# UZ-SLAMLab/DefSLAM

Measured on AMD Instinct MI355X. Metric: SfT GN iters/sec (500-node mesh, 1k matches), higher is better.
Workload: dtype f64

## Files before the change

### defslam_amd/csrc/sft_batch.h

```cpp
#pragma once

#define SFTB_NW 8
#ifndef SFTB_LIN_NW
#define SFTB_LIN_NW 8
#endif
#ifndef SFTB_LIN_WAVES
#define SFTB_LIN_WAVES 2
#endif
#ifndef SFTB_TRIAL_WAVES
#define SFTB_TRIAL_WAVES 2
#endif

__device__ __forceinline__ void sftb_ctl_lds(char* smem, Ctl*& ctl, double*& red, double*& out, double*& panel) {
  ctl = reinterpret_cast<Ctl*>(smem);
  red = reinterpret_cast<double*>(smem + 512);
  out = red + 16 * 27 + 5;
  panel = out + 32;
}

__global__ __launch_bounds__(64 * SFTB_NW, 2) void sftb_init_kernel(const SftDev* __restrict__ probs, SftRun* __restrict__ runs, int* __restrict__ counters, int* __restrict__ lin_list, int tail_below) {
  const SftDev& P = probs[blockIdx.x];
  if (blockIdx.x == 0 && threadIdx.x == 0 && (int)gridDim.x <= tail_below) counters[6] = 1;
  init_state<64 * SFTB_NW>(P);
  if (threadIdx.x == 0) {
    SftRun& R = runs[blockIdx.x];
    R.lambda = -1.0; R.ni = 2.0; R.chi_cur = 0.0; R.chi_ini = 0.0; R.rho = 0.0; R.lambda_start = 0.0;
    R.it = 0; R.qmax = 0; R.nbad = 0; R.accepted = 0; R.all_ok = 1; R.iters = 0; R.trials = 0; R.fact_ok = 1;
    R.state = P.max_iters > 0 ? SFTB_LIN : SFTB_FINISH;
    if (P.max_iters > 0) lin_list[atomicAdd(&counters[2], 1)] = blockIdx.x;
  }
}

template <int NW>
__device__ __forceinline__ void sftb_lin_problem(const SftDev& P, SftRun& R, Ctl* ctl, double* red, double* out, double* panel) {
  constexpr int NT = 64 * NW;
  const int tid = threadIdx.x;
  auto nothing = [] {};
  const double chi0 = linearise<NW, decltype(nothing), true>(P, ctl, red, out, panel, nothing);
  double lambda = R.lambda;
  if (R.it == 0) {
    double mx = 0.0;
    for (int r = tid; r < P.Dn; r += NT) mx = fmax(mx, fabs(h_diag(P, r)));
    if (tid < 6) mx = fmax(mx, fabs(P.Hcorner[tid * 8]));
    mx = block_max(mx, red);
    lambda = 1e-5 * mx;
  }
  if (tid == 0) {
    if (R.it == 0) { R.lambda = lambda; R.ni = 2.0; R.nbad = 0; }
    R.chi_cur = chi0; R.chi_ini = chi0; R.qmax = 0; R.rho = 0.0; R.accepted = 0; R.all_ok = 1; R.lambda_start = lambda;
    R.state = SFTB_TRIAL;
  }
}

__global__ __launch_bounds__(64 * SFTB_LIN_NW, SFTB_LIN_WAVES) void sftb_lin_kernel(const SftDev* __restrict__ probs, SftRun* __restrict__ runs, int* __restrict__ counters,
                                                                                  const int* __restrict__ lin_list, int B, int tail_below) {
  constexpr int NW = SFTB_LIN_NW, NT = 64 * NW;
  extern __shared__ __attribute__((aligned(16))) char smem[];
  __shared__ int next_b;
  Ctl* ctl; double *red, *out, *panel;
  sftb_ctl_lds(smem, ctl, red, out, panel);
  const int tid = threadIdx.x;
  if (counters[6] || B - counters[0] <= tail_below) {
    if (blockIdx.x == 0 && tid == 0) counters[6] = 1;
    return;
  }
  if (blockIdx.x == 0 && tid == 0) counters[7]++;
  auto fetch = [&]() { const int i = atomicAdd(&counters[3], 1); return i < counters[2] ? lin_list[i] : -1; };
  int nxt = -1;
  if (tid == 0) nxt = fetch();
  while (true) {
    if (tid == 0) next_b = nxt;
    __syncthreads();
    const int b = __builtin_amdgcn_readfirstlane(next_b);
    if (b < 0) break;
    if (tid == 0) { nxt = fetch(); atomicAdd(&counters[9], 1); }
    sftb_lin_problem<NW>(probs[b], runs[b], ctl, red, out, panel);
  }
}

__global__ __launch_bounds__(64, 1) void sftb_factor_kernel(const SftDev* __restrict__ probs, SftRun* __restrict__ runs, int* __restrict__ counters, int B) {
  extern __shared__ __attribute__((aligned(16))) char smem[];
  lds_double* lds = to_lds(reinterpret_cast<double*>(smem));
  const int lane = threadIdx.x;
  if (counters[6]) return;
  for (int i = lane; i < WV_LDS_DOUBLES; i += 64) lds[i] = 0.0;
  if (blockIdx.x == 0 && lane == 0) { counters[2] = 0; counters[3] = 0; }
  WvPrev Q;
  Q.Lg = nullptr; Q.Linv = nullptr; Q.x = nullptr; Q.nT = 0; Q.active = 0; Q.xb = 0.0;
  int n_done = 0;
  while (true) {
    int b = 0;
    if (lane == 0) b = atomicAdd(&counters[1], 1);
    b = __builtin_amdgcn_readfirstlane(b);
    if (b >= B) break;
    if (runs[b].state != SFTB_TRIAL) continue;
    const SftDev& P = probs[b];
    const double lambda = runs[b].lambda;
    double xcam;
    const int ok = wv_factor(P, lambda, lambda, lds, Q, xcam);
    if (lane == 0) runs[b].fact_ok = ok;
    Q = wv_prev_of(P, ok, xcam, lane);
    n_done++;
  }
  int lane_now;
  asm volatile("v_mbcnt_lo_u32_b32 %0, -1, 0\n\tv_mbcnt_hi_u32_b32 %0, -1, %0" : "=v"(lane_now));
  if (Q.active) wv_backsub_now(Q, lane_now);
  if (lane_now == 0 && n_done) atomicAdd(&counters[8], n_done);
}

template <int NW>
__device__ __forceinline__ int sftb_trial_problem(const SftDev& P, SftRun& R, Ctl* ctl, double* red, double* out, double* panel, int* counters, int* lin_list, int b) {
  constexpr int NT = 64 * NW;
  const int tid = threadIdx.x;
  const int Dn = P.Dn;
  const int Dnp = ((Dn + NB - 1) / NB) * NB;
  const int ok = R.fact_ok;
  const double lam = R.lambda;
  const bool in_lds = P.lds_class >= 1;
  if (!in_lds)
    for (int i = tid; i < 3 * P.n; i += NT) {
      const double v = P.xyz[i];
      P.xyz_bak[i] = v;
      const int a = P.act[i / 3];
      if (a >= 0) P.xyz[i] = v + P.x[3 * a + (i % 3)];
    }
  if (tid < 7) R.pose_bak[tid] = P.pose[tid];
  __syncthreads();
  if (tid == 0) pose_oplus(P.pose, P.x + Dnp);
  double sc = 0.0;
  for (int r = tid; r < Dn; r += NT) { const double xv = P.x[r]; sc += xv * (lam * xv + P.Hbord[(size_t)6 * Dnp + r]); }
  if (tid < 6) { const double xv = P.x[Dnp + tid]; sc += xv * (lam * xv + P.Hcorner[42 + tid]); }
  __syncthreads();
  block_sum<1>(&sc, red, out);
  const double scale = out[0];
  __syncthreads();
  const auto staged = asm_records<NW, 1>(P, panel);
  const double chi_new = in_lds ? eval_edges<false, 1>(P, ctl, red, out, staged, P.x)
                                : eval_edges<false, 0>(P, ctl, red, out, asm_records<NW, 0>(P, panel));
  if (tid == 0) {
    const double tempChi = ok ? chi_new : DBL_MAX;
    double rho = (R.chi_cur - tempChi);
    rho /= (scale + 1e-3);
    R.rho = rho;
    if (rho > 0 && isfinite(tempChi)) {
      double alpha = 1. - pow((2 * rho - 1), 3);
      alpha = fmin(alpha, 2. / 3.);
      const double sf = fmax(1. / 3., alpha);
      R.lambda = lam * sf; R.ni = 2.0; R.chi_cur = tempChi; R.accepted = 1;
      ctl->stop = 0;
    } else {
      R.lambda = lam * R.ni; R.ni *= 2.0;
      ctl->stop = 1;
    }
    R.qmax++;
    R.all_ok &= ok;
    ctl->qmax = R.qmax;
    ctl->rho = rho;
  }
  __syncthreads();
  if (ctl->stop) {
    if (!in_lds)
      for (int i = tid; i < 3 * P.n; i += NT) P.xyz[i] = P.xyz_bak[i];
    if (tid < 7) P.pose[tid] = R.pose_bak[tid];
  } else if (in_lds) {
    for (int i = tid; i < 3 * P.n; i += NT) P.xyz[i] = staged.xyz_l[i];
  }
  const bool again = (ctl->rho < 0) && (ctl->qmax < 10);
  if (again) return 0;
  __syncthreads();
  if (tid == 0) {
    const int qmax = R.qmax;
// ... 101 lines not shown
```

### defslam_amd/csrc/sft_wave.h

```cpp
#pragma once

#if defined(WV_STEP_TRACE) && defined(DSH_LAB)
#define WV_T_DECL long long wv_tr[9] = {0, 0, 0, 0, 0, 0, 0, 0, 0}, wv_tl = clock64()
#define WV_T(e) do { const long long t__ = clock64(); wv_tr[e] += t__ - wv_tl; wv_tl = t__; } while (0)
#define WV_T_ARG , long long (&wv_tr)[9], long long& wv_tl
#define WV_T_PASS , wv_tr, wv_tl
#define WV_T_DUMP(P) do { if ((threadIdx.x & 63) == 0) for (int e__ = 0; e__ < 9; e__++) (P).dbg[40 + e__] = (double)wv_tr[e__]; } while (0)
#else
#define WV_T_DECL do {} while (0)
#define WV_T(e) do {} while (0)
#define WV_T_ARG
#define WV_T_PASS
#define WV_T_DUMP(P) do {} while (0)
#endif

__host__ __device__ constexpr int wv_phys(int r, int d) {
  return d == 0 ? r : (d <= 3 ? 8 * d + r : (d == 4 ? 32 + (r & 3) : 8 * (8 - d) + ((r + 8 - d) & 7)));
}
constexpr int WV_AGPR_TILES = 32;
constexpr int WV_L_WIN = 0;
constexpr int WV_L_BORD = 1024;
constexpr int WV_L_WSCR = 2048;
constexpr int WV_L_CN = 2336;
constexpr int WV_L_XRING = 2400;
// ... 145 lines not shown
struct WvB2 { double n0, n1; };
struct WvBO { double v[4][2]; };
__device__ __forceinline__ WvB2 wv_bq_load(const lds_double* tile, int lane) {
  const v2d_w a = reinterpret_cast<const lds_v2d*>(tile)[lane];
  return WvB2{a.x, a.y};
}
__device__ __forceinline__ void wv_bq_store(lds_double* tile, int lane, const WvB2& v) {
  reinterpret_cast<lds_v2d*>(tile)[lane] = (v2d_w){v.n0, v.n1};
}
__device__ __forceinline__ int wv_bo_lane(int lane) { return (lane & 0x30) | (lane & 3); }
__device__ __forceinline__ void wv_bo_load(const lds_double* tile, int lane, WvBO& o) {
  const lds_v2d* p = reinterpret_cast<const lds_v2d*>(tile) + wv_bo_lane(lane);
#pragma unroll
  for (int q = 0; q < 4; q++) { const v2d_w a = p[4 * q]; o.v[q][0] = a.x; o.v[q][1] = a.y; }
}
__device__ __forceinline__ void wv_upd_b4(WvB2& C, const v4d& A, const WvBO& B, int q0 = 0) {
#define WV_MF(q) asm volatile("v_mfma_f64_4x4x4_4b_f64 %0, %2, %3, %0 neg:[1,0,0]\n\tv_mfma_f64_4x4x4_4b_f64 %1, %2, %4, %1 neg:[1,0,0]" \
                              : "+v"(C.n0), "+v"(C.n1) : "v"(A[q]), "v"(B.v[q][0]), "v"(B.v[q][1]) : "memory")
  asm volatile("s_nop 1" : "+v"(C.n0), "+v"(C.n1));
  if (q0 <= 0) WV_MF(0);
  if (q0 <= 1) WV_MF(1);
  if (q0 <= 2) WV_MF(2);
  WV_MF(3);
#undef WV_MF
}
__device__ __forceinline__ void wv_trsm_b4(WvB2& Y, const v4d& Wt, const WvBO& B) {
  asm volatile("s_nop 1\n\t"
               "v_mfma_f64_4x4x4_4b_f64 %0, %2, %6, 0\n\t"
               "v_mfma_f64_4x4x4_4b_f64 %1, %2, %7, 0\n\t"
               "v_mfma_f64_4x4x4_4b_f64 %0, %3, %8, %0\n\t"
               "v_mfma_f64_4x4x4_4b_f64 %1, %3, %9, %1\n\t"
               "v_mfma_f64_4x4x4_4b_f64 %0, %4, %10, %0\n\t"
               "v_mfma_f64_4x4x4_4b_f64 %1, %4, %11, %1\n\t"
               "v_mfma_f64_4x4x4_4b_f64 %0, %5, %12, %0\n\t"
               "v_mfma_f64_4x4x4_4b_f64 %1, %5, %13, %1"
               : "=&v"(Y.n0), "=&v"(Y.n1)
               : "v"(Wt[0]), "v"(Wt[1]), "v"(Wt[2]), "v"(Wt[3]), "v"(B.v[0][0]), "v"(B.v[0][1]), "v"(B.v[1][0]), "v"(B.v[1][1]), "v"(B.v[2][0]), "v"(B.v[2][1]),
                 "v"(B.v[3][0]), "v"(B.v[3][1])
               : "memory");
}
__device__ __forceinline__ int wv_bstd_index(int lane) { return 2 * wv_bo_lane(lane) + ((lane >> 2) & 1); }

template <int CTRL>
__device__ __forceinline__ double wv_dpp_mov(double v) {
  const int lo = __builtin_amdgcn_mov_dpp(__double2loint(v), CTRL, 0xF, 0xF, false);
  const int hi = __builtin_amdgcn_mov_dpp(__double2hiint(v), CTRL, 0xF, 0xF, false);
  return __hiloint2double(hi, lo);
}

__device__ __forceinline__ bool wv_chol_inv(v4d& a, v4d& w) {
  const int lane = threadIdx.x & 63;
  const int g = lane >> 4, c = lane & 15;
  w = (v4d){(g == c) ? 1.0 : 0.0, (g + 4 == c) ? 1.0 : 0.0, (g + 8 == c) ? 1.0 : 0.0, (g + 12 == c) ? 1.0 : 0.0};
  double plast = 1.0;
#pragma unroll
  for (int J = 0; J < 4; J++) {
    const double aJ = a[J];
    const double sel = chol4_inverse_operand(aJ, J, g, c & 3, plast);
    const double wJ = w[J];
    double zw, lp;
    if (J < 3) {
      asm volatile("s_nop 1\n\t"
                   "v_mfma_f64_4x4x4_4b_f64 %0, %2, %3, 0\n\t"
                   "v_mfma_f64_4x4x4_4b_f64 %1, %2, %4, 0\n\t"
                   "s_nop 7"
                   : "=&v"(zw), "=&v"(lp)
                   : "v"(sel), "v"(wJ), "v"(aJ));
      const double nlp = -lp;
      const double below = (c >= 4 * J + 4) ? nlp : 0.0;
      asm volatile("s_nop 1\n\t"
                   "v_mfma_f64_16x16x4_f64 %0, %2, %3, %0\n\t"
                   "v_mfma_f64_16x16x4_f64 %1, %4, %5, %1\n\t" WV_NOP_MFMA_RESULT
                   : "+v"(a), "+v"(w)
                   : "v"(nlp), "v"(lp), "v"(below), "v"(zw));
      w[J] = zw;
    } else {
      asm volatile("s_nop 1\n\tv_mfma_f64_4x4x4_4b_f64 %0, %1, %2, 0\n\ts_nop 7" : "=&v"(zw) : "v"(sel), "v"(wJ));
      w[J] = zw;
    }
  }
  return plast > 0.0;
}

struct WvProb {
  int Dn, Dnp, nT, q8;
  double lambda, lam_corner;
  unsigned bofs;
  const SFT_G double* Hc;
  const SFT_G uint32_t* hgl;
  const SFT_G double* Hbord;
  SFT_G double *Lg, *Linv;
};

typedef unsigned v4u_w __attribute__((ext_vector_type(4)));
__device__ __forceinline__ void wv_list(const WvProb& W, int I, int d, int lane, unsigned (&o)[4]) {
  const SFT_G v4u_w* row = reinterpret_cast<const SFT_G v4u_w*>(W.hgl + ((size_t)(I < W.nT ? I : W.nT) * (BT + 1) + d) * 256);
  const v4u_w v = row[lane];
  o[0] = v.x; o[1] = v.y; o[2] = v.z; o[3] = v.w;
}
__device__ __forceinline__ v4d wv_gather_vgpr(const WvProb& W, const unsigned (&o)[4]) {
  const auto b8 = reinterpret_cast<const SFT_G char*>(W.Hc);
  v4d v;
#pragma unroll
  for (int q = 0; q < 4; q++) v[q] = *reinterpret_cast<const SFT_G double*>(b8 + o[q]);
  return v;
}
__device__ __forceinline__ WvB2 wv_border_fresh(const WvProb& W, int J, int lane) {
  const SFT_G double* p = W.Hbord + TS * (J < W.nT ? J : W.nT);
  (void)lane;
  return WvB2{p[W.bofs], p[W.bofs + 4 * (unsigned)W.Dnp]};
}

struct WvRowList { unsigned o[8][4]; };
__device__ __forceinline__ void wv_row_list(const WvProb& W, int I, int lane, WvRowList& L) {
#pragma unroll
  for (int d = 0; d < 8; d++) wv_list(W, I, d, lane, L.o[d]);
}
template <int PH, int D>
__device__ __forceinline__ void wv_row_fetch_d(const WvProb& W, const WvRowList& L, int dmax, v4d& fresh4) {
  if constexpr (D < 8) {
    if (D <= dmax) {
      if constexpr (D == 4) fresh4 = wv_gather_vgpr(W, L.o[D]);
      else wv_gather_agpr<wv_phys(PH, D)>(W.Hc, L.o[D][0], L.o[D][1], L.o[D][2], L.o[D][3]);
    }
    wv_row_fetch_d<PH, D + 1>(W, L, dmax, fresh4);
  }
}

struct WvPrev {
  const SFT_G double* Lg;
  const SFT_G double* Linv;
  SFT_G double* x;
  int nT, active;
  double xb;
};
__device__ __forceinline__ void wv_bs_request(const WvPrev& Q, int J, lds_double* land, int lane) {
  const unsigned voff = 16u * (unsigned)lane;
  const SFT_G char* col = reinterpret_cast<const SFT_G char*>(Q.Lg + ((size_t)J * (BT + 1)) * 256);
  const SFT_G char* w = reinterpret_cast<const SFT_G char*>(Q.Linv + (size_t)J * 256);
  const unsigned l0 = (unsigned)__builtin_amdgcn_readfirstlane((int)(size_t)land);
  asm volatile("s_mov_b32 m0, %2\n\ts_nop 0\n\t"
               "global_load_lds_dwordx4 %0, %1\n\t"
               "global_load_lds_dwordx4 %0, %1 offset:2048\n\t"
               "global_load_lds_dwordx4 %0, %1 offset:3072"
               :: "v"(voff), "s"(col), "s"(l0) : "memory", "m0");
#pragma unroll
  for (int grp = 1; grp < 5; grp++) {
    const SFT_G char* cg = col + 4096 * grp;
    const unsigned lg = l0 + 4096u * grp;
    if (grp < 4)
      asm volatile("s_mov_b32 m0, %2\n\ts_nop 0\n\t"
                   "global_load_lds_dwordx4 %0, %1\n\t"
                   "global_load_lds_dwordx4 %0, %1 offset:1024\n\t"
                   "global_load_lds_dwordx4 %0, %1 offset:2048\n\t"
                   "global_load_lds_dwordx4 %0, %1 offset:3072"
                   :: "v"(voff), "s"(cg), "s"(lg) : "memory", "m0");
    else
      asm volatile("s_mov_b32 m0, %2\n\ts_nop 0\n\t"
                   "global_load_lds_dwordx4 %0, %1\n\t"
                   "global_load_lds_dwordx4 %0, %1 offset:1024"
                   :: "v"(voff), "s"(cg), "s"(lg) : "memory", "m0");
  }
  asm volatile("s_mov_b32 m0, %2\n\ts_nop 0\n\t"
               "global_load_lds_dwordx4 %0, %1\n\t"
               "global_load_lds_dwordx4 %0, %1 offset:1024"
               :: "v"(voff), "s"(w), "s"(l0 + 18u * 1024u) : "memory", "m0");
}
__device__ __forceinline__ void wv_bs_column(const WvPrev& Q, int J, const lds_double* land, lds_double* xring, int lane) {
  const int c = lane & 15;
  const lds_v2d* t2 = reinterpret_cast<const lds_v2d*>(land) + 2 * lane;
  double s[4];
  {
    const lds_double* tb = land + wv_bstd_index(lane);
    s[0] = tb[0] * Q.xb; s[1] = tb[8] * Q.xb; s[2] = tb[16] * Q.xb; s[3] = tb[24] * Q.xb;
  }
#pragma unroll
  for (int d = 1; d <= 8; d++) {
    const double xr = xring[((J + d) & 7) * 16 + c];
    const v2d_w a = t2[128 * d], b = t2[128 * d + 1];
    s[0] = fma(a.x, xr, s[0]); s[1] = fma(a.y, xr, s[1]); s[2] = fma(b.x, xr, s[2]); s[3] = fma(b.y, xr, s[3]);
  }
#pragma unroll
  for (int q = 0; q < 4; q++) {
    s[q] += wv_dpp_mov<0x128>(s[q]);
    s[q] += wv_dpp_mov<0x124>(s[q]);
    s[q] += wv_dpp_mov<0x122>(s[q]);
    s[q] += wv_dpp_mov<0x121>(s[q]);
  }
  const v2d_w wa = t2[128 * 9], wb = t2[128 * 9 + 1];
  double p = wa.x * -s[0];
  p = fma(wa.y, -s[1], p); p = fma(wb.x, -s[2], p); p = fma(wb.y, -s[3], p);
  p = sum_rows(p);
  if (lane < TS) { xring[(J & 7) * 16 + lane] = p; Q.x[TS * J + lane] = p; }
}
__device__ __forceinline__ void wv_bs_step(const WvPrev& Q, int J, lds_double* lds, int lane) {
  wv_bs_column(Q, J, lds + WV_L_LAND, lds + WV_L_XRING, lane);
  asm volatile("s_waitcnt lgkmcnt(0)" ::: "memory");
  if (J >= 1) wv_bs_request(Q, J - 1, lds + WV_L_LAND, lane);
}
__device__ __forceinline__ void wv_bs_begin(const WvPrev& Q, lds_double* lds, int lane) {
  lds_double* xring = lds + WV_L_XRING;
  xring[lane] = 0.0; xring[64 + lane] = 0.0;
  wv_bs_request(Q, Q.nT - 1, lds + WV_L_LAND, lane);
}
__device__ __forceinline__ void wv_backsub_now(const WvPrev& Q, int lane) {
  const int c = lane & 15;
  (void)c;
  double xr[8];
#pragma unroll
  for (int s = 0; s < 8; s++) xr[s] = 0.0;
  struct Col { v4d t[10]; };
  auto fetch = [&](int J) -> Col {
    Col C;
    if (J >= 0) {
      const SFT_G double* col = Q.Lg + ((size_t)J * (BT + 1)) * 256 + 4 * lane;
#pragma unroll
      for (int i = 1; i <= 8; i++) C.t[i] = (J + i < Q.nT) ? *reinterpret_cast<const SFT_G v4d*>(col + 256 * i) : (v4d){0.0, 0.0, 0.0, 0.0};
      {
        const SFT_G double* tb = col - 4 * lane + wv_bstd_index(lane);
        C.t[0] = (v4d){tb[0], tb[8], tb[16], tb[24]};
      }
      C.t[9] = *reinterpret_cast<const SFT_G v4d*>(Q.Linv + (size_t)J * 256 + 4 * lane);
    } else {
#pragma unroll
      for (int i = 0; i < 10; i++) C.t[i] = (v4d){0.0, 0.0, 0.0, 0.0};
    }
    return C;
  };
  auto solve_col = [&](const Col& C, int J, auto phc) {
    constexpr int ph = decltype(phc)::value;
    double s[4];
#pragma unroll
    for (int q = 0; q < 4; q++) s[q] = C.t[0][q] * Q.xb;
#pragma unroll
    for (int dd = 1; dd <= 8; dd++)
#pragma unroll
      for (int q = 0; q < 4; q++) s[q] = fma(C.t[dd][q], xr[(ph + dd) & 7], s[q]);
#pragma unroll
    for (int q = 0; q < 4; q++) {
      s[q] += wv_dpp_mov<0x128>(s[q]);
      s[q] += wv_dpp_mov<0x124>(s[q]);
      s[q] += wv_dpp_mov<0x122>(s[q]);
      s[q] += wv_dpp_mov<0x121>(s[q]);
    }
    double p = C.t[9][0] * -s[0];
#pragma unroll
    for (int q = 1; q < 4; q++) p = fma(C.t[9][q], -s[q], p);
    p = sum_rows(p);
    xr[ph] = p;
    if (lane < TS) Q.x[TS * J + lane] = p;
  };
  int J = Q.nT - 1;
  Col c0 = fetch(J), c1 = fetch(J - 1);
#pragma unroll 1
  for (; J >= 0; J -= 2) {
    const Col n0 = fetch(J - 2), n1 = fetch(J - 3);
    switch (J & 7) {
      case 7: solve_col(c0, J, std::integral_constant<int, 7>{}); solve_col(c1, J - 1, std::integral_constant<int, 6>{}); break;
      case 5: solve_col(c0, J, std::integral_constant<int, 5>{}); solve_col(c1, J - 1, std::integral_constant<int, 4>{}); break;
      case 3: solve_col(c0, J, std::integral_constant<int, 3>{}); solve_col(c1, J - 1, std::integral_constant<int, 2>{}); break;
      default: solve_col(c0, J, std::integral_constant<int, 1>{}); solve_col(c1, J - 1, std::integral_constant<int, 0>{}); break;
    }
    c0 = n0; c1 = n1;
  }
}

struct WvState {
  v4d Y[9];
  WvB2 Yq;
  WvBO Yo;
  double corner;
  v4d araw;
  WvB2 bnext;
  WvRowList rl;
  unsigned al[4];
  unsigned off_lane, off_bord;
  int ok;
};

template <int PH, int I, int IEND>
__device__ __forceinline__ void wv_trsm_cols(WvState& S, const WvTri& Wt, int k, int nT, const v4d& D4, int lane) {
  if constexpr (I <= IEND) {
    (void)k; (void)nT;
    if constexpr (I == 4) {
      wv_trsm4_vgpr(S.Y[4], Wt, D4);
    } else {
      wv_trsm4_agpr<wv_phys((PH + I) & 7, I)>(S.Y[I], Wt);
    }
    wv_trsm_cols<PH, I + 1, IEND>(S, Wt, k, nT, D4, lane);
  }
}

__host__ __device__ constexpr int wv_tile_index(int I, int J) {
  int n = 0;
  for (int i = 1; i <= 7; i++)
    for (int j = 1; j <= i; j++) {
      if (i == I && j == J) return n;
      if (i - j != 4) n++;
    }
  return n;
}
template <int PH, int SLOT>
__device__ __forceinline__ void wv_fetch_slot(const WvProb& W, const WvRowList& L) {
  if constexpr (SLOT < 28) {
    constexpr int t = SLOT / 4, q = SLOT % 4, d = t < 4 ? t : t + 1;
    wv_gather1_agpr<wv_phys(PH, d), q>(W.Hc, L.o[d][q]);
  }
}
template <int PH, bool TAIL, int I, int J>
__device__ __forceinline__ void wv_update_tiles(const WvProb& W, WvState& S, int k, int nT, int q8, SFT_G double* col) {
  if constexpr (I <= 8) {
    constexpr int d = I - J, r = (PH + I) & 7;
    if constexpr (d != 4) {
      if (!TAIL || k + I < nT) wv_upd_agpr<wv_phys(r, d)>(S.Y[J], S.Y[I], (I == 8) ? q8 : 0);
      if constexpr (I <= 7) {
        constexpr int n = wv_tile_index(I, J);
        if constexpr (n < 18) {
          const SFT_G double* slot = col + 256 * (n >> 1);
          if constexpr (n == 0) {
            const v2d_w yb = (v2d_w){S.Yq.n0, S.Yq.n1};
            asm volatile("global_store_dwordx4 %0, %1, %2" :: "v"(S.off_bord), "v"(yb), "s"(slot) : "memory");
          } else if constexpr (n >= 2) {
            const v4d& y = S.Y[n >> 1];
            const v2d_w half = (v2d_w){y[2 * (n & 1)], y[2 * (n & 1) + 1]};
            asm volatile("global_store_dwordx4 %0, %1, %2 offset:%c3" :: "v"(S.off_lane), "v"(half), "s"(slot), "n"(16 * (n & 1)) : "memory");
          }
        }
        wv_fetch_slot<PH, 2 * n>(W, S.rl);
        wv_fetch_slot<PH, 2 * n + 1>(W, S.rl);
      }
    }
    if constexpr (J < I) wv_update_tiles<PH, TAIL, I, J + 1>(W, S, k, nT, q8, col);
  }
}
template <int PH, bool TAIL, int I0, int I1>
__device__ __forceinline__ void wv_update_rows(const WvProb& W, WvState& S, int k, int nT, int q8, SFT_G double* col) {
  if constexpr (I0 <= I1) {
    wv_update_tiles<PH, TAIL, I0, 1>(W, S, k, nT, q8, col);
    wv_update_rows<PH, TAIL, I0 + 1, I1>(W, S, k, nT, q8, col);
  }
}
template <int PH, int T>
__device__ __forceinline__ lds_double* wv_task_tile(lds_double* lds) {
  if constexpr (T < 7) return lds + WV_L_BORD + 128 * ((PH + T + 1) & 7);
  else if constexpr (T < 10) return lds + WV_L_WIN + 256 * (wv_phys((PH + T - 2) & 7, 4) - WV_AGPR_TILES);
  else if constexpr (T == 10) return lds + WV_L_BORD + 128 * (PH & 7);
  else return lds + WV_L_WIN + 256 * (wv_phys(PH & 7, 4) - WV_AGPR_TILES);
}
template <int T> struct WvTaskTile { using type = typename std::conditional<(T < 7 || T == 10), WvB2, v4d>::type; };
template <int T> using wv_task_t = typename WvTaskTile<T>::type;
template <int PH, int T>
__device__ __forceinline__ wv_task_t<T> wv_task_load(lds_double* lds, int lane) {
  if constexpr (T < 7 || T == 10) return wv_bq_load(wv_task_tile<PH, T>(lds), lane);
  else return wv_lds_load(wv_task_tile<PH, T>(lds), lane);
}
template <int PH, int T>
__device__ __forceinline__ void wv_task_store(lds_double* lds, int lane, const wv_task_t<T>& C) {
  if constexpr (T < 7 || T == 10) wv_bq_store(wv_task_tile<PH, T>(lds), lane, C);
  else wv_lds_store(wv_task_tile<PH, T>(lds), lane, C);
}
template <int T>
__device__ __forceinline__ void wv_task_mfma(wv_task_t<T>& C, const WvState& S, int q8) {
  if constexpr (T < 7) wv_upd_b4(C, S.Y[T + 1], S.Yo);
  else if constexpr (T < 10) wv_upd_vgpr(C, S.Y[T - 6], S.Y[T - 2]);
  else if constexpr (T == 10) wv_upd_b4(C, S.Y[8], S.Yo, q8);
  else wv_upd_vgpr(C, S.Y[4], S.Y[8], q8);
}
template <int PH, int T, int TEND>
__device__ __forceinline__ void wv_lds_pipe_next(const WvState& S, int q8, lds_double* lds, int lane, wv_task_t<T>& C, const wv_task_t<T - 1>& Cprev) {
  if constexpr (T < TEND) {
    wv_task_t<T + 1> Cn = wv_task_load<PH, T + 1>(lds, lane);
    wv_task_mfma<T>(C, S, q8);
    wv_task_store<PH, T - 1>(lds, lane, Cprev);
    wv_lds_pipe_next<PH, T + 1, TEND>(S, q8, lds, lane, Cn, C);
  } else {
    wv_task_mfma<T>(C, S, q8);
    wv_task_store<PH, T - 1>(lds, lane, Cprev);
    wv_mfma_fence();
    wv_task_store<PH, T>(lds, lane, C);
  }
}
template <int PH, int T0, int TEND>
__device__ __forceinline__ void wv_lds_pipe(const WvState& S, int q8, lds_double* lds, int lane) {
  wv_task_t<T0> C = wv_task_load<PH, T0>(lds, lane);
  wv_task_t<T0 + 1> Cn = wv_task_load<PH, T0 + 1>(lds, lane);
  wv_task_mfma<T0>(C, S, q8);
  wv_lds_pipe_next<PH, T0 + 1, TEND>(S, q8, lds, lane, Cn, C);
}

template <int PH>
__device__ __forceinline__ v4d wv_step_diag(const WvProb& W, int k, int lane) {
  v4d d = wv_read_agpr<wv_phys(PH, 0)>();
  const int g = lane >> 4, c = lane & 15;
#pragma unroll
  for (int q = 0; q < 4; q++)
    if (g + 4 * q == c && TS * k + c < W.Dn) d[q] += W.lambda;
  return d;
}

template <int PH, bool TAIL>
__device__ __forceinline__ void wv_step_rest(const WvProb& W, WvState& S, const v4d& w, int k, lds_double* lds, int lane, const WvPrev& Q WV_T_ARG) {
  lds_double* ldsw = lds + WV_L_WIN;
  lds_double* ldsb = lds + WV_L_BORD;
  lds_double* wscr = lds + WV_L_WSCR;
  const int nT = W.nT;
  WvBO Bk;
  wv_bo_load(ldsb + 128 * PH, lane, Bk);
  const v4d D4 = wv_lds_load(ldsw + 256 * (wv_phys((PH + 4) & 7, 4) - WV_AGPR_TILES), lane);
// ... 21 lines not shown
#pragma unroll
    for (int q = 0; q < 4; q++) { yba[q] = ta[8 * q]; ybs[q] = tb[8 * q]; }
  }
  asm volatile("" :: "v"(D4[0]), "v"(D4[1]), "v"(D4[2]), "v"(D4[3]));
  wv_trsm_cols<PH, 5, 7>(S, Wq, k, nT, D4, lane);
  if (W.q8 == 1) wv_trsm4_vgpr_q1(S.Y[8], Wq, S.araw);
  else wv_trsm_vgpr(S.Y[8], Wt, S.araw, W.q8);
  wv_mfma_fence();
  WV_T(3);
  SFT_G double* col = W.Lg + ((size_t)k * (BT + 1)) * 256;
  v4d fresh4 = wv_gather_vgpr(W, S.rl.o[4]);
  asm volatile("" : "+v"(S.bnext.n0), "+v"(S.bnext.n1));
  wv_bq_store(ldsb + 128 * PH, lane, S.bnext);
  WV_T(4);
  asm volatile("s_nop 1\n\t"
               "v_mfma_f64_4x4x4_4b_f64 %0, %1, %5, %0 neg:[1,0,0]\n\ts_nop 3\n\t"
               "v_mfma_f64_4x4x4_4b_f64 %0, %2, %6, %0 neg:[1,0,0]\n\ts_nop 3\n\t"
               "v_mfma_f64_4x4x4_4b_f64 %0, %3, %7, %0 neg:[1,0,0]\n\ts_nop 3\n\t"
               "v_mfma_f64_4x4x4_4b_f64 %0, %4, %8, %0 neg:[1,0,0]"
               : "+v"(S.corner)
               : "v"(yba[0]), "v"(yba[1]), "v"(yba[2]), "v"(yba[3]), "v"(ybs[0]), "v"(ybs[1]), "v"(ybs[2]), "v"(ybs[3])
               : "memory");
  wv_update_rows<PH, TAIL, 1, 7>(W, S, k, nT, W.q8, col);
  wv_lds_pipe<PH, 0, 9>(S, W.q8, lds, lane);
  WV_T(5);
  wv_wait_vm();
  WV_T(6);
  {
    WvB2 C10 = wv_task_load<PH, 10>(lds, lane);
    wv_update_rows<PH, TAIL, 8, 8>(W, S, k, nT, W.q8, col);
    wv_task_mfma<10>(C10, S, W.q8);
    wv_task_mfma<11>(fresh4, S, W.q8);
    wv_task_store<PH, 10>(lds, lane, C10);
    wv_mfma_fence();
    wv_task_store<PH, 11>(lds, lane, fresh4);
  }
  asm volatile("" : "+v"(S.corner));
  WV_T(8);
}

struct WvTriList { unsigned o[36][4]; };
template <int R, int D>
__device__ __forceinline__ void wv_prologue_lists(const WvProb& W, int lane, WvTriList& T) {
  if constexpr (R < 8) {
    wv_list(W, R, D, lane, T.o[R * (R + 1) / 2 + D]);
    if constexpr (D < R) wv_prologue_lists<R, D + 1>(W, lane, T);
    else wv_prologue_lists<R + 1, 0>(W, lane, T);
  }
}
template <int R, int D>
__device__ __forceinline__ void wv_prologue_gathers(const WvProb& W, WvTriList& T, v4d (&f4)[8]) {
  if constexpr (R < 8) {
    unsigned (&o)[4] = T.o[R * (R + 1) / 2 + D];
    if constexpr (R == 0 && D == 0) {
#pragma unroll
      for (int t = 0; t < 36; t++) asm volatile("" : "+v"(T.o[t][0]), "+v"(T.o[t][1]), "+v"(T.o[t][2]), "+v"(T.o[t][3]));
    }
    if constexpr (D == 4) f4[R] = wv_gather_vgpr(W, o);
    else wv_gather_agpr<wv_phys(R, D)>(W.Hc, o[0], o[1], o[2], o[3]);
    if constexpr (D < R) wv_prologue_gathers<R, D + 1>(W, T, f4);
    else wv_prologue_gathers<R + 1, 0>(W, T, f4);
  }
}
template <int PH>
__device__ __forceinline__ void wv_prologue_store(lds_double* lds, int lane, v4d& f4, WvB2& bd) {
  if constexpr (PH >= 4) {
    asm volatile("" : "+v"(f4));
    wv_lds_store(lds + WV_L_WIN + 256 * (wv_phys(PH, 4) - WV_AGPR_TILES), lane, f4);
  }
  asm volatile("" : "+v"(bd.n0), "+v"(bd.n1));
  wv_bq_store(lds + WV_L_BORD + 128 * PH, lane, bd);
}

__device__ __forceinline__ int wv_factor(const SftDev& P, double lambda, double lam_corner, lds_double* lds, const WvPrev& Q, double& xcam_out) {
  asm volatile("" ::: "a0", "a255");
  int lane;
  asm volatile("v_mbcnt_lo_u32_b32 %0, -1, 0\n\tv_mbcnt_hi_u32_b32 %0, -1, %0" : "=v"(lane));
  const int g = lane >> 4, c = lane & 15;
  WvProb W;
  W.Dn = uni(P.Dn);
  W.Dnp = ((W.Dn + NB - 1) / NB) * NB;
  W.nT = W.Dnp / TS;
  W.q8 = min(3, max(0, (TS * BT - uni(P.kd)) / 4));
  W.lambda = lambda;
  W.lam_corner = lam_corner;
  W.bofs = (unsigned)((c & 3) * W.Dnp + 4 * (c >> 2) + g);
  W.Hc = uni(P.Hc); W.hgl = uni(P.hgatherT); W.Hbord = uni(P.Hbord); W.Lg = uni(P.Lb); W.Linv = uni(P.Linv);
  lds_double* wscr = lds + WV_L_WSCR;
  lds_double* Cn = lds + WV_L_CN;
#ifdef DSH_LAB
  const long long wv_t0 = clock64();
#endif
  if (Q.active) wv_bs_begin(Q, lds, lane);
  WvState S;
#pragma unroll
  for (int i = 0; i < 9; i++) S.Y[i] = (v4d){0.0, 0.0, 0.0, 0.0};
  const int cr = 4 * (c >> 3) + g, cc = 4 * ((c >> 2) & 1) + (c & 3);
  S.corner = 0.0;
  if (cr < SFT_BORDER && cc < SFT_BORDER && cc <= cr) S.corner = P.Hcorner[cr * 7 + cc] + ((cr == cc && cr < 6) ? lam_corner : 0.0);
  S.ok = 1;
  {
    WvTriList T;
    v4d f4[8];
    WvB2 bd[8];
    wv_prologue_lists<0, 0>(W, lane, T);
    wv_prologue_gathers<0, 0>(W, T, f4);
#pragma unroll
    for (int r = 0; r < 8; r++) bd[r] = wv_border_fresh(W, r, lane);
    wv_list(W, 8, 8, lane, S.al);
    wv_prologue_store<0>(lds, lane, f4[0], bd[0]); wv_prologue_store<1>(lds, lane, f4[1], bd[1]); wv_prologue_store<2>(lds, lane, f4[2], bd[2]);
    wv_prologue_store<3>(lds, lane, f4[3], bd[3]); wv_prologue_store<4>(lds, lane, f4[4], bd[4]); wv_prologue_store<5>(lds, lane, f4[5], bd[5]);
    wv_prologue_store<6>(lds, lane, f4[6], bd[6]); wv_prologue_store<7>(lds, lane, f4[7], bd[7]);
  }
  wv_wait_vm();
  asm volatile("" : "+v"(S.al[0]), "+v"(S.al[1]), "+v"(S.al[2]), "+v"(S.al[3]));
#ifdef DSH_LAB
  const long long wv_t1 = clock64();
  const long long wv_w1 = wall_clock64();
#endif

  WV_T_DECL;
#pragma unroll 1
  for (int k = 0; k < W.nT; k++) {
    const int ph = k & 7;
    asm volatile("v_lshlrev_b32 %0, 5, %1" : "=v"(S.off_lane) : "v"(lane));
    asm volatile("v_lshlrev_b32 %0, 4, %1" : "=v"(S.off_bord) : "v"(lane));
    S.araw = wv_gather_vgpr(W, S.al);
    wv_list(W, k + 9, 8, lane, S.al);
    wv_row_list(W, k + 8, lane, S.rl);
    S.bnext = wv_border_fresh(W, k + 8, lane);
    v4d d;
    switch (ph) {
      case 0: d = wv_step_diag<0>(W, k, lane); break;
      case 1: d = wv_step_diag<1>(W, k, lane); break;
      case 2: d = wv_step_diag<2>(W, k, lane); break;
      case 3: d = wv_step_diag<3>(W, k, lane); break;
      case 4: d = wv_step_diag<4>(W, k, lane); break;
      case 5: d = wv_step_diag<5>(W, k, lane); break;
      case 6: d = wv_step_diag<6>(W, k, lane); break;
      default: d = wv_step_diag<7>(W, k, lane); break;
    }
    WV_T(0);
    if (Q.active) {
      const int J = Q.nT - 1 - k;
      if (J >= 0) wv_bs_step(Q, J, lds, lane);
    }
    WV_T(7);
    v4d w;
    if (!wv_chol_inv(d, w)) {
#ifdef DSH_LAB
      if (S.ok && lane == 0) P.dbg[3] = 1000.0 + k;
#endif
      S.ok = 0;
    }
    WV_T(1);
    {
      const SFT_G double* slot = W.Linv + (size_t)k * 256;
      const v2d_w w01 = (v2d_w){w[0], w[1]}, w23 = (v2d_w){w[2], w[3]};
      asm volatile("global_store_dwordx4 %0, %1, %3\n\tglobal_store_dwordx4 %0, %2, %3 offset:16" :: "v"(S.off_lane), "v"(w01), "v"(w23), "s"(slot) : "memory");
    }
    switch (ph + ((k + 8 >= W.nT) ? 8 : 0)) {
      case 0: wv_step_rest<0, false>(W, S, w, k, lds, lane, Q WV_T_PASS); break;
      case 1: wv_step_rest<1, false>(W, S, w, k, lds, lane, Q WV_T_PASS); break;
      case 2: wv_step_rest<2, false>(W, S, w, k, lds, lane, Q WV_T_PASS); break;
      case 3: wv_step_rest<3, false>(W, S, w, k, lds, lane, Q WV_T_PASS); break;
      case 4: wv_step_rest<4, false>(W, S, w, k, lds, lane, Q WV_T_PASS); break;
      case 5: wv_step_rest<5, false>(W, S, w, k, lds, lane, Q WV_T_PASS); break;
      case 6: wv_step_rest<6, false>(W, S, w, k, lds, lane, Q WV_T_PASS); break;
      case 7: wv_step_rest<7, false>(W, S, w, k, lds, lane, Q WV_T_PASS); break;
      case 8: wv_step_rest<0, true>(W, S, w, k, lds, lane, Q WV_T_PASS); break;
      case 9: wv_step_rest<1, true>(W, S, w, k, lds, lane, Q WV_T_PASS); break;
      case 10: wv_step_rest<2, true>(W, S, w, k, lds, lane, Q WV_T_PASS); break;
      case 11: wv_step_rest<3, true>(W, S, w, k, lds, lane, Q WV_T_PASS); break;
      case 12: wv_step_rest<4, true>(W, S, w, k, lds, lane, Q WV_T_PASS); break;
      case 13: wv_step_rest<5, true>(W, S, w, k, lds, lane, Q WV_T_PASS); break;
      case 14: wv_step_rest<6, true>(W, S, w, k, lds, lane, Q WV_T_PASS); break;
      default: wv_step_rest<7, true>(W, S, w, k, lds, lane, Q WV_T_PASS); break;
    }
  }
  WV_T_DUMP(P);
  if (Q.active) {
    for (int J = Q.nT - 1 - W.nT; J >= 0; J--) { wv_wait_vm(); wv_bs_step(Q, J, lds, lane); }
  }
#ifdef DSH_LAB
  const long long wv_t2 = clock64();
  const long long wv_w2 = wall_clock64();
#endif
  wv_mfma_fence();
  {
    int l2;
    asm volatile("v_mbcnt_lo_u32_b32 %0, -1, 0\n\tv_mbcnt_hi_u32_b32 %0, -1, %0" : "=v"(l2));
    const int g2 = l2 >> 4, c2 = l2 & 15;
    const int cr2 = 4 * (c2 >> 3) + g2, cc2 = 4 * ((c2 >> 2) & 1) + (c2 & 3);
    if (cr2 < SFT_BORDER && cc2 < SFT_BORDER) Cn[cr2 * 7 + cc2] = S.corner;
  }
  double xcam = 0.0;
  {
    int okc = 1;
    if (lane == 0) {
      double xc[6] = {0, 0, 0, 0, 0, 0};
      bool bad = false;
      for (int kk = 0; kk < 6; kk++) {
        double dd = Cn[kk * 7 + kk];
        for (int j = 0; j < kk; j++) dd -= Cn[kk * 7 + j] * Cn[kk * 7 + j];
        if (!(dd > 0.0)) bad = true;
        const double piv = sqrt(dd);
        Cn[kk * 7 + kk] = piv;
        for (int r = kk + 1; r < 7; r++) {
          double v = Cn[r * 7 + kk];
          for (int j = 0; j < kk; j++) v -= Cn[r * 7 + j] * Cn[kk * 7 + j];
          Cn[r * 7 + kk] = v / piv;
        }
      }
      if (bad) okc = 0;
      for (int kk = 5; kk >= 0; kk--) {
        double v = Cn[6 * 7 + kk];
        for (int r = kk + 1; r < 6; r++) v -= Cn[r * 7 + kk] * xc[r];
        xc[kk] = v / Cn[kk * 7 + kk];
      }
      for (int kk = 0; kk < 6; kk++) Cn[49 + kk] = xc[kk];
    }
    okc = __builtin_amdgcn_readfirstlane(okc);
    if (!okc) S.ok = 0;
    if (c < 6) xcam = Cn[49 + c];
  }
  xcam_out = xcam;
#ifdef DSH_LAB
  if (lane == 0) { P.dbg[5] = (double)(wv_t1 - wv_t0); P.dbg[6] = (double)(wv_t2 - wv_t1); P.dbg[4] = (double)(wv_w2 - wv_w1); }
#endif
  return __builtin_amdgcn_readfirstlane(S.ok);
}

__device__ __forceinline__ WvPrev wv_prev_of(const SftDev& P, int ok, double xcam, int lane_) {
  (void)lane_;
  int lane;
  asm volatile("v_mbcnt_lo_u32_b32 %0, -1, 0\n\tv_mbcnt_hi_u32_b32 %0, -1, %0" : "=v"(lane));
  const int c = lane & 15;
  WvPrev Q;
  const int Dn = uni(P.Dn), Dnp = ((Dn + NB - 1) / NB) * NB;
  Q.Lg = uni(P.Lb); Q.Linv = uni(P.Linv); Q.x = uni(P.x);
  Q.nT = Dnp / TS;
  Q.active = ok;
  Q.xb = (c < 6) ? xcam : ((c == 6) ? -1.0 : 0.0);
  if (ok && lane < 6) P.x[Dnp + lane] = xcam;
  return Q;
}

__device__ __forceinline__ int wv_factor_solve(const SftDev& P, double lambda, double lam_corner, lds_double* lds) {
  WvPrev none;
  none.Lg = nullptr; none.Linv = nullptr; none.x = nullptr; none.nT = 0; none.active = 0; none.xb = 0.0;
  double xcam;
  const int ok = wv_factor(P, lambda, lam_corner, lds, none, xcam);
  int lane;
  asm volatile("v_mbcnt_lo_u32_b32 %0, -1, 0\n\tv_mbcnt_hi_u32_b32 %0, -1, %0" : "=v"(lane));
  const WvPrev Q = wv_prev_of(P, ok, xcam, lane);
#ifdef DSH_LAB
  const long long t2 = clock64();
#endif
  if (ok) wv_backsub_now(Q, lane);
#ifdef DSH_LAB
  if (lane == 0) P.dbg[7] = (double)(clock64() - t2);
#endif
  return ok;
}
```

Baseline: 415,600.

## Store factor tiles as split half-tiles and skip zero granules with exec masks

Changes the global layout of stored Cholesky tiles: each lane now writes two 16-byte halves 1024 bytes apart instead of a contiguous 32-byte chunk, and the load-to-LDS and register backsubstitution readers are updated to match. Stores and loads for the border tile and the inverse-diagonal tile are masked by per-granule exec masks, so structurally zero entries are neither written nor read. Tail tiles past nT are skipped, and the LDS landing area is pre-zeroed so masked loads read zeros. The intent is to cut global memory traffic and use more coalesced accesses in factorization and backsubstitution, at the cost of extra exec-mask manipulation and more layout-dependent code that must stay consistent between writer and readers.

```diff
diff --git a/defslam_amd/csrc/sft_batch.h b/defslam_amd/csrc/sft_batch.h
--- a/defslam_amd/csrc/sft_batch.h
+++ b/defslam_amd/csrc/sft_batch.h
@@ -86,7 +86,7 @@
   for (int i = lane; i < WV_LDS_DOUBLES; i += 64) lds[i] = 0.0;
   if (blockIdx.x == 0 && lane == 0) { counters[2] = 0; counters[3] = 0; }
   WvPrev Q;
-  Q.Lg = nullptr; Q.Linv = nullptr; Q.x = nullptr; Q.nT = 0; Q.active = 0; Q.xb = 0.0;
+  Q.Lg = nullptr; Q.Linv = nullptr; Q.x = nullptr; Q.nT = 0; Q.active = 0; Q.m8[0] = Q.m8[1] = 0; Q.xb = 0.0;
   int n_done = 0;
   while (true) {
     int b = 0;
diff --git a/defslam_amd/csrc/sft_wave.h b/defslam_amd/csrc/sft_wave.h
--- a/defslam_amd/csrc/sft_wave.h
+++ b/defslam_amd/csrc/sft_wave.h
@@ -251,8 +251,19 @@
   return plast > 0.0;
 }
 
+__host__ __device__ constexpr unsigned long long wv_granule_mask(int t) {
+  unsigned long long m = 0;
+  for (int g = 0; g < 4; g++) {
+    const int n = t + g + 1 < 0 ? 0 : (t + g + 1 > 16 ? 16 : t + g + 1);
+    m |= ((1ull << n) - 1ull) << (16 * g);
+  }
+  return m;
+}
+constexpr unsigned long long WV_MASK_W0 = wv_granule_mask(4), WV_MASK_W1 = wv_granule_mask(12);
+
 struct WvProb {
   int Dn, Dnp, nT, q8;
+  unsigned long long m8[2];
   double lambda, lam_corner;
   unsigned bofs;
   const SFT_G double* Hc;
@@ -301,6 +312,7 @@
   const SFT_G double* Linv;
   SFT_G double* x;
   int nT, active;
+  unsigned long long m8[2];
   double xb;
 };
 __device__ __forceinline__ void wv_bs_request(const WvPrev& Q, int J, lds_double* land, int lane) {
@@ -308,36 +320,54 @@
   const SFT_G char* col = reinterpret_cast<const SFT_G char*>(Q.Lg + ((size_t)J * (BT + 1)) * 256);
   const SFT_G char* w = reinterpret_cast<const SFT_G char*>(Q.Linv + (size_t)J * 256);
   const unsigned l0 = (unsigned)__builtin_amdgcn_readfirstlane((int)(size_t)land);
-  asm volatile("s_mov_b32 m0, %2\n\ts_nop 0\n\t"
-               "global_load_lds_dwordx4 %0, %1\n\t"
-               "global_load_lds_dwordx4 %0, %1 offset:2048\n\t"
-               "global_load_lds_dwordx4 %0, %1 offset:3072"
-               :: "v"(voff), "s"(col), "s"(l0) : "memory", "m0");
-#pragma unroll
-  for (int grp = 1; grp < 5; grp++) {
-    const SFT_G char* cg = col + 4096 * grp;
-    const unsigned lg = l0 + 4096u * grp;
-    if (grp < 4)
+  unsigned long long keep;
+  if (J + 8 < Q.nT) {
+    asm volatile("s_mov_b32 m0, %2\n\ts_nop 0\n\t"
+                 "global_load_lds_dwordx4 %0, %1\n\t"
+                 "global_load_lds_dwordx4 %0, %1 offset:2048\n\t"
+                 "global_load_lds_dwordx4 %0, %1 offset:3072"
+                 :: "v"(voff), "s"(col), "s"(l0) : "memory", "m0");
+#pragma unroll
+    for (int grp = 1; grp < 4; grp++) {
+      const SFT_G char* cg = col + 4096 * grp;
+      const unsigned lg = l0 + 4096u * grp;
       asm volatile("s_mov_b32 m0, %2\n\ts_nop 0\n\t"
                    "global_load_lds_dwordx4 %0, %1\n\t"
                    "global_load_lds_dwordx4 %0, %1 offset:1024\n\t"
                    "global_load_lds_dwordx4 %0, %1 offset:2048\n\t"
                    "global_load_lds_dwordx4 %0, %1 offset:3072"
                    :: "v"(voff), "s"(cg), "s"(lg) : "memory", "m0");
-    else
-      asm volatile("s_mov_b32 m0, %2\n\ts_nop 0\n\t"
-                   "global_load_lds_dwordx4 %0, %1\n\t"
-                   "global_load_lds_dwordx4 %0, %1 offset:1024"
-                   :: "v"(voff), "s"(cg), "s"(lg) : "memory", "m0");
-  }
-  asm volatile("s_mov_b32 m0, %2\n\ts_nop 0\n\t"
-               "global_load_lds_dwordx4 %0, %1\n\t"
-               "global_load_lds_dwordx4 %0, %1 offset:1024"
-               :: "v"(voff), "s"(w), "s"(l0 + 18u * 1024u) : "memory", "m0");
+    }
+    asm volatile("s_mov_b32 m0, %3\n\ts_nop 0\n\t"
+                 "s_and_saveexec_b64 %0, %4\n\t"
+                 "global_load_lds_dwordx4 %1, %2\n\t"
+                 "s_mov_b64 exec, %0\n\t"
+                 "s_and_saveexec_b64 %0, %5\n\t"
+                 "global_load_lds_dwordx4 %1, %2 offset:1024\n\t"
+                 "s_mov_b64 exec, %0"
+                 : "=&s"(keep) : "v"(voff), "s"(col + 16384), "s"(l0 + 16384u), "s"(Q.m8[0]), "s"(Q.m8[1]) : "memory", "m0", "scc");
+  } else {
+    asm volatile("s_mov_b32 m0, %2\n\ts_nop 0\n\tglobal_load_lds_dwordx4 %0, %1" :: "v"(voff), "s"(col), "s"(l0) : "memory", "m0");
+#pragma unroll
+    for (int i = 1; i < 8; i++)
+      if (J + i < Q.nT)
+        asm volatile("s_mov_b32 m0, %2\n\ts_nop 0\n\t"
+                     "global_load_lds_dwordx4 %0, %1\n\t"
+                     "global_load_lds_dwordx4 %0, %1 offset:1024"
+                     :: "v"(voff), "s"(col + 2048 * i), "s"(l0 + 2048u * i) : "memory", "m0");
+  }
+  asm volatile("s_mov_b32 m0, %3\n\ts_nop 0\n\t"
+               "s_and_saveexec_b64 %0, %4\n\t"
+               "global_load_lds_dwordx4 %1, %2\n\t"
+               "s_mov_b64 exec, %0\n\t"
+               "s_and_saveexec_b64 %0, %5\n\t"
+               "global_load_lds_dwordx4 %1, %2 offset:1024\n\t"
+               "s_mov_b64 exec, %0"
+               : "=&s"(keep) : "v"(voff), "s"(w), "s"(l0 + 18u * 1024u), "s"(WV_MASK_W0), "s"(WV_MASK_W1) : "memory", "m0", "scc");
 }
 __device__ __forceinline__ void wv_bs_column(const WvPrev& Q, int J, const lds_double* land, lds_double* xring, int lane) {
   const int c = lane & 15;
-  const lds_v2d* t2 = reinterpret_cast<const lds_v2d*>(land) + 2 * lane;
+  const lds_v2d* t2 = reinterpret_cast<const lds_v2d*>(land) + lane;
   double s[4];
   {
     const lds_double* tb = land + wv_bstd_index(lane);
@@ -346,7 +376,7 @@
 #pragma unroll
   for (int d = 1; d <= 8; d++) {
     const double xr = xring[((J + d) & 7) * 16 + c];
-    const v2d_w a = t2[128 * d], b = t2[128 * d + 1];
+    const v2d_w a = t2[128 * d], b = t2[128 * d + 64];
     s[0] = fma(a.x, xr, s[0]); s[1] = fma(a.y, xr, s[1]); s[2] = fma(b.x, xr, s[2]); s[3] = fma(b.y, xr, s[3]);
   }
 #pragma unroll
@@ -356,7 +386,7 @@
     s[q] += wv_dpp_mov<0x122>(s[q]);
     s[q] += wv_dpp_mov<0x121>(s[q]);
   }
-  const v2d_w wa = t2[128 * 9], wb = t2[128 * 9 + 1];
+  const v2d_w wa = t2[128 * 9], wb = t2[128 * 9 + 64];
   double p = wa.x * -s[0];
   p = fma(wa.y, -s[1], p); p = fma(wb.x, -s[2], p); p = fma(wb.y, -s[3], p);
   p = sum_rows(p);
@@ -370,6 +400,12 @@
 __device__ __forceinline__ void wv_bs_begin(const WvPrev& Q, lds_double* lds, int lane) {
   lds_double* xring = lds + WV_L_XRING;
   xring[lane] = 0.0; xring[64 + lane] = 0.0;
+  {
+    lds_v2d* z = reinterpret_cast<lds_v2d*>(lds + WV_L_LAND + 256) + lane;
+#pragma unroll
+    for (int i = 0; i < 16; i++) z[64 * i] = (v2d_w){0.0, 0.0};
+    asm volatile("s_waitcnt lgkmcnt(0)" ::: "memory");
+  }
   wv_bs_request(Q, Q.nT - 1, lds + WV_L_LAND, lane);
 }
 __device__ __forceinline__ void wv_backsub_now(const WvPrev& Q, int lane) {
@@ -382,14 +418,21 @@
   auto fetch = [&](int J) -> Col {
     Col C;
     if (J >= 0) {
-      const SFT_G double* col = Q.Lg + ((size_t)J * (BT + 1)) * 256 + 4 * lane;
-#pragma unroll
-      for (int i = 1; i <= 8; i++) C.t[i] = (J + i < Q.nT) ? *reinterpret_cast<const SFT_G v4d*>(col + 256 * i) : (v4d){0.0, 0.0, 0.0, 0.0};
+      const SFT_G double* col = Q.Lg + ((size_t)J * (BT + 1)) * 256;
+      auto slot = [&](const SFT_G double* t, bool in0, bool in1) -> v4d {
+        const v2d_w zero = (v2d_w){0.0, 0.0};
+        const v2d_w a = in0 ? *reinterpret_cast<const SFT_G v2d_w*>(t + 2 * lane) : zero;
+        const v2d_w b = in1 ? *reinterpret_cast<const SFT_G v2d_w*>(t + 128 + 2 * lane) : zero;
+        return (v4d){a.x, a.y, b.x, b.y};
+      };
+#pragma unroll
+      for (int i = 1; i <= 7; i++) { const bool in = J + i < Q.nT; C.t[i] = slot(col + 256 * i, in, in); }
+      C.t[8] = slot(col + 256 * 8, J + 8 < Q.nT && ((Q.m8[0] >> lane) & 1), J + 8 < Q.nT && ((Q.m8[1] >> lane) & 1));
       {
-        const SFT_G double* tb = col - 4 * lane + wv_bstd_index(lane);
+        const SFT_G double* tb = col + wv_bstd_index(lane);
         C.t[0] = (v4d){tb[0], tb[8], tb[16], tb[24]};
       }
-      C.t[9] = *reinterpret_cast<const SFT_G v4d*>(Q.Linv + (size_t)J * 256 + 4 * lane);
+      C.t[9] = slot(Q.Linv + (size_t)J * 256, (WV_MASK_W0 >> lane) & 1, (WV_MASK_W1 >> lane) & 1);
     } else {
 #pragma unroll
       for (int i = 0; i < 10; i++) C.t[i] = (v4d){0.0, 0.0, 0.0, 0.0};
@@ -443,7 +486,7 @@
   WvB2 bnext;
   WvRowList rl;
   unsigned al[4];
-  unsigned off_lane, off_bord;
+  unsigned off_lane;
   int ok;
 };
 
@@ -488,11 +531,19 @@
           const SFT_G double* slot = col + 256 * (n >> 1);
           if constexpr (n == 0) {
             const v2d_w yb = (v2d_w){S.Yq.n0, S.Yq.n1};
-            asm volatile("global_store_dwordx4 %0, %1, %2" :: "v"(S.off_bord), "v"(yb), "s"(slot) : "memory");
+            asm volatile("global_store_dwordx4 %0, %1, %2" :: "v"(S.off_lane), "v"(yb), "s"(slot) : "memory");
           } else if constexpr (n >= 2) {
             const v4d& y = S.Y[n >> 1];
             const v2d_w half = (v2d_w){y[2 * (n & 1)], y[2 * (n & 1) + 1]};
-            asm volatile("global_store_dwordx4 %0, %1, %2 offset:%c3" :: "v"(S.off_lane), "v"(half), "s"(slot), "n"(16 * (n & 1)) : "memory");
+            if constexpr ((n >> 1) == 8) {
+              if constexpr (!TAIL) {
+                unsigned long long keep;
+                asm volatile("s_and_saveexec_b64 %0, %4\n\tglobal_store_dwordx4 %1, %2, %3 offset:%c5\n\ts_mov_b64 exec, %0"
+                             : "=&s"(keep) : "v"(S.off_lane), "v"(half), "s"(slot), "s"(W.m8[n & 1]), "n"(1024 * (n & 1)) : "memory", "scc");
+              }
+            } else if (!TAIL || k + (n >> 1) < nT) {
+              asm volatile("global_store_dwordx4 %0, %1, %2 offset:%c3" :: "v"(S.off_lane), "v"(half), "s"(slot), "n"(1024 * (n & 1)) : "memory");
+            }
           }
         }
         wv_fetch_slot<PH, 2 * n>(W, S.rl);
@@ -680,6 +731,8 @@
   W.Dnp = ((W.Dn + NB - 1) / NB) * NB;
   W.nT = W.Dnp / TS;
   W.q8 = min(3, max(0, (TS * BT - uni(P.kd)) / 4));
+  W.m8[0] = wv_granule_mask(4 - (TS * BT - uni(P.kd)));
+  W.m8[1] = wv_granule_mask(12 - (TS * BT - uni(P.kd)));
   W.lambda = lambda;
   W.lam_corner = lam_corner;
   W.bofs = (unsigned)((c & 3) * W.Dnp + 4 * (c >> 2) + g);
@@ -721,8 +774,7 @@
 #pragma unroll 1
   for (int k = 0; k < W.nT; k++) {
     const int ph = k & 7;
-    asm volatile("v_lshlrev_b32 %0, 5, %1" : "=v"(S.off_lane) : "v"(lane));
-    asm volatile("v_lshlrev_b32 %0, 4, %1" : "=v"(S.off_bord) : "v"(lane));
+    asm volatile("v_lshlrev_b32 %0, 4, %1" : "=v"(S.off_lane) : "v"(lane));
     S.araw = wv_gather_vgpr(W, S.al);
     wv_list(W, k + 9, 8, lane, S.al);
     wv_row_list(W, k + 8, lane, S.rl);
@@ -755,7 +807,10 @@
     {
       const SFT_G double* slot = W.Linv + (size_t)k * 256;
       const v2d_w w01 = (v2d_w){w[0], w[1]}, w23 = (v2d_w){w[2], w[3]};
-      asm volatile("global_store_dwordx4 %0, %1, %3\n\tglobal_store_dwordx4 %0, %2, %3 offset:16" :: "v"(S.off_lane), "v"(w01), "v"(w23), "s"(slot) : "memory");
+      unsigned long long keep;
+      asm volatile("s_and_saveexec_b64 %0, %5\n\tglobal_store_dwordx4 %1, %2, %4\n\ts_mov_b64 exec, %0\n\t"
+                   "s_and_saveexec_b64 %0, %6\n\tglobal_store_dwordx4 %1, %3, %4 offset:1024\n\ts_mov_b64 exec, %0"
+                   : "=&s"(keep) : "v"(S.off_lane), "v"(w01), "v"(w23), "s"(slot), "s"(WV_MASK_W0), "s"(WV_MASK_W1) : "memory", "scc");
     }
     switch (ph + ((k + 8 >= W.nT) ? 8 : 0)) {
       case 0: wv_step_rest<0, false>(W, S, w, k, lds, lane, Q WV_T_PASS); break;
@@ -838,6 +893,8 @@
   const int Dn = uni(P.Dn), Dnp = ((Dn + NB - 1) / NB) * NB;
   Q.Lg = uni(P.Lb); Q.Linv = uni(P.Linv); Q.x = uni(P.x);
   Q.nT = Dnp / TS;
+  Q.m8[0] = wv_granule_mask(4 - (TS * BT - uni(P.kd)));
+  Q.m8[1] = wv_granule_mask(12 - (TS * BT - uni(P.kd)));
   Q.active = ok;
   Q.xb = (c < 6) ? xcam : ((c == 6) ? -1.0 : 0.0);
   if (ok && lane < 6) P.x[Dnp + lane] = xcam;
@@ -846,7 +903,7 @@
 
 __device__ __forceinline__ int wv_factor_solve(const SftDev& P, double lambda, double lam_corner, lds_double* lds) {
   WvPrev none;
-  none.Lg = nullptr; none.Linv = nullptr; none.x = nullptr; none.nT = 0; none.active = 0; none.xb = 0.0;
+  none.Lg = nullptr; none.Linv = nullptr; none.x = nullptr; none.nT = 0; none.active = 0; none.m8[0] = none.m8[1] = 0; none.xb = 0.0;
   double xcam;
   const int ok = wv_factor(P, lambda, lam_corner, lds, none, xcam);
   int lane;
```

New measurement: 425,200, median of 6. 2.3% higher.
